# borangundogan/PPO-2DGrid

Hardware: AMD Instinct MI355X
Metric: env-steps/sec (rollout+GAE+PPO update), 4096 envs, 16x16 mediumhard (higher is better)
Workload: dtype fp32

## Files before the change

include/merlin_hip.h:

```cpp
#ifndef MERLIN_HIP_H
#define MERLIN_HIP_H

#include <stdint.h>

#ifdef __cplusplus
extern "C" {
#endif

#define MERLIN_ABI_VERSION 3

#define MERLIN_OK 0
#define MERLIN_E_INVALID 1
#define MERLIN_E_HIP 2
#define MERLIN_E_DEVICE 3
#define MERLIN_E_UNSUPPORTED 4

#define MERLIN_EASY 0
#define MERLIN_MEDIUM 1
#define MERLIN_MEDIUMHARD 2
#define MERLIN_HARD 3
#define MERLIN_HARDEST 4

#define MERLIN_DEVERR_BAD_ACTION 1u
#define MERLIN_DEVERR_PLACE_OBJ 2u
// ... 42 lines not shown
                    double *ep_return_dev, int32_t *ep_length_dev, int32_t autoreset,
                    void *stream);
int merlin_env_act_step(merlin_env *env, const float *head_part_dev, int32_t n_parts, const float *b_actor_dev,
                        const float *b_critic_dev, int32_t act_dim, int32_t deterministic, uint64_t seed,
                        const int64_t *epoch_dev, int64_t step, int64_t env_offset, int64_t *action_dev,
                        float *logp_dev, float *value_dev, uint32_t *obs_dev, float *reward_dev,
                        uint8_t *terminated_dev, uint8_t *truncated_dev, float *done_dev, double *ep_return_dev,
                        int32_t *ep_length_dev, void *stream);
int merlin_group_act(const uint32_t *codes_dev, int32_t groups, const float *T2_dev, const float *b2_dev,
                     const float *W3t_dev, const float *b3_dev, const float *W4p_dev, const float *b4_dev,
                     const float *Wa_dev, const float *ba_dev, const float *Wc_dev, const float *bc_dev,
                     int32_t act_dim, float *a3_ws_dev, float *head_part_dev, int32_t shared_weights, void *stream);
int merlin_env_set_refill_interval(merlin_env *env, int32_t every);
int merlin_env_refill(merlin_env *env, void *stream);
int merlin_env_set_step_fallback(merlin_env *env, int32_t on);
int merlin_env_full_obs(merlin_env *env, uint8_t *out_dev, void *stream);
int merlin_env_get_state(merlin_env *env, uint32_t *walls_host, int32_t *agent_host,
                         uint64_t *rng_host, void *stream);
#define MERLIN_FRAME_TILES 22
int merlin_frame_atlas(int32_t tile_size, uint8_t *out_host);
int merlin_render_frames(const uint32_t *walls_dev, const int32_t *goal_dev, const int32_t *agent_dev,
                         const int32_t *map_index_dev, int64_t n_frames, int32_t size, int32_t tile_size,
                         int32_t highlight, uint8_t *out_dev, void *stream);
int merlin_env_render(merlin_env *env, const int64_t *index_dev, int64_t n, int32_t tile_size,
                      int32_t highlight, uint8_t *out_dev, void *stream);
int merlin_env_snapshot(merlin_env *env, uint32_t *walls_dev, int32_t *goal_dev, int32_t *agent_dev,
                        void *stream);
int merlin_shortest_paths(const uint32_t *walls_dev, const int32_t *goal_dev, const int32_t *agent_dev,
                          const int32_t *map_index_dev, int64_t n, int32_t size, int32_t *dist_dev,
                          int16_t *field_dev, void *stream);
// ... 264 lines not shown
```

ppo-2dgrid_amd/csrc/merlin_capi.hip:

```cpp
#include <math.h>
#include <string.h>

#include <mutex>
#include <string>
#include <vector>

#include <algorithm>

#include "merlin_internal.h"

struct merlin_env {
    merlin::EnvDev dev;
    int device;
    bool has_state;
    int steps_since_refill;
    int refill_every;
    bool no_fallback = false;
    bool seed_slots_full = false;
    uint8_t *diff_buf = nullptr;
};

namespace {

thread_local std::string g_err;
// ... 438 lines not shown
        if (err == hipSuccess) err = hipMemset(*p, 0, bytes);
    };
    alloc((void **)&d.walls, n * d.sp * sizeof(uint32_t));
    alloc((void **)&d.agent, n * sizeof(uint4));
    alloc((void **)&d.rng_s, n * sizeof(ulonglong2));
    alloc((void **)&d.rng_i, n * sizeof(ulonglong2));
    alloc((void **)&d.rng_b, n * sizeof(uint2));
    alloc((void **)&d.ep_ret, n * sizeof(double));
    alloc((void **)&d.ep_len, n * sizeof(int32_t));
    alloc((void **)&d.err, 2 * sizeof(uint32_t));
    alloc((void **)&d.pg_walls, n * d.sp * sizeof(uint32_t));
    alloc((void **)&d.pg_agent, n * sizeof(uint4));
    alloc((void **)&d.pg_rng_s, n * sizeof(ulonglong2));
    alloc((void **)&d.pg_rng_b, n * sizeof(uint2));
    alloc((void **)&d.pg_valid, n * sizeof(uint8_t));
    alloc((void **)&d.rflag, n * sizeof(uint8_t));
    alloc((void **)&d.bflag, (n + 63) / 64);
    if (d.explore_on) alloc((void **)&d.visited, n * d.sp * sizeof(uint32_t));
    alloc((void **)&e->diff_buf, n * sizeof(uint8_t));
    if (err != hipSuccess) {
        merlin_env_destroy(e);
        return hip_fail(err, "hipMalloc(env state)");
    }
    *out = e;
    return MERLIN_OK;
}

int merlin_env_destroy(merlin_env *e) {
    if (!e) return MERLIN_OK;
    merlin::EnvDev &d = e->dev;
    void *ptrs[] = {d.walls, d.agent, d.rng_s, d.rng_i, d.rng_b, d.ep_ret, d.ep_len, d.err, d.visited,
                    d.pg_walls, d.pg_agent, d.pg_rng_s, d.pg_rng_b, d.pg_valid, d.rflag, d.bflag, e->diff_buf};
    for (void *p : ptrs)
        if (p) (void)hipFree(p);
    delete e;
    return MERLIN_OK;
}

int merlin_env_num_envs(const merlin_env *e) { return e ? e->dev.n : -1; }
int merlin_env_size(const merlin_env *e) { return e ? e->dev.size : -1; }

int merlin_env_seed(merlin_env *e, const uint64_t *seeds, int32_t n, void *stream) {
    if (!e || !seeds) return fail(MERLIN_E_INVALID, "null argument");
    if (n != e->dev.n) return fail(MERLIN_E_INVALID, "seed count must equal num_envs");
    hipStream_t s = (hipStream_t)stream;
    const size_t N = (size_t)n;
    ulonglong2 *st = new ulonglong2[N];
    ulonglong2 *inc = new ulonglong2[N];
    for (size_t i = 0; i < N; i++) {
        U128 a, b;
        seed_pcg64(seeds[i], a, b);
        st[i] = make_ulonglong2(a.lo, a.hi);
        inc[i] = make_ulonglong2(b.lo, b.hi);
    }
    hipError_t err = hipMemcpyAsync(e->dev.rng_s, st, N * sizeof(ulonglong2), hipMemcpyHostToDevice, s);
    if (err == hipSuccess)
        err = hipMemcpyAsync(e->dev.rng_i, inc, N * sizeof(ulonglong2), hipMemcpyHostToDevice, s);
    if (err == hipSuccess) err = merlin::zero_async(e->dev.rng_b, N * sizeof(uint2), s);
    if (err == hipSuccess) err = merlin::zero_async(e->dev.pg_valid, N, s);
    e->seed_slots_full = false;
    if (err == hipSuccess) err = hipStreamSynchronize(s);
    delete[] st;
    delete[] inc;
    if (err != hipSuccess) return hip_fail(err, "merlin_env_seed");
    return MERLIN_OK;
}

int merlin_env_set_difficulties(merlin_env *e, const int32_t *diff, int32_t n, void *stream) {
    if (!e) return fail(MERLIN_E_INVALID, "null env");
    hipStream_t s = (hipStream_t)stream;
    const size_t N = (size_t)e->dev.n;
    hipError_t err = hipSuccess;
    uint8_t *host = nullptr;
    if (diff) {
        if (n != e->dev.n) return fail(MERLIN_E_INVALID, "difficulty count must equal num_envs");
        for (size_t i = 0; i < N; i++) {
            if (diff[i] < MERLIN_EASY || diff[i] > MERLIN_HARDEST) return fail(MERLIN_E_INVALID, "unknown difficulty");
            if (diff[i] == MERLIN_HARDEST && e->dev.size < 8)
                return fail(MERLIN_E_UNSUPPORTED, "hardest needs size >= 8 (integers(2, size/2 - 1) is empty below)");
        }
        host = new uint8_t[N];
        for (size_t i = 0; i < N; i++) host[i] = (uint8_t)diff[i];
        err = hipMemcpyAsync(e->diff_buf, host, N, hipMemcpyHostToDevice, s);
        e->dev.diff = e->diff_buf;
    } else {
        e->dev.diff = nullptr;
    }
    if (err == hipSuccess) err = merlin::zero_async(e->dev.pg_valid, N, s);
    e->seed_slots_full = false;
    if (err == hipSuccess) err = hipStreamSynchronize(s);
    delete[] host;
    if (err != hipSuccess) return hip_fail(err, "merlin_env_set_difficulties");
    return MERLIN_OK;
}

int merlin_env_reset(merlin_env *e, const uint8_t *mask, uint32_t *obs, void *stream) {
    if (!e) return fail(MERLIN_E_INVALID, "null env");
    HIP_TRY(merlin::launch_env_reset(e->dev, mask, obs, (hipStream_t)stream));
    e->steps_since_refill = 0;
    if (!mask) {
        e->has_state = true;
        e->seed_slots_full = e->dev.reseed != 0;
    }
    return MERLIN_OK;
}

int merlin_env_step(merlin_env *e, const int64_t *actions, int32_t n_steps, int64_t action_stride,
                    uint32_t *obs, float *reward, uint8_t *term, uint8_t *trunc, float *done,
                    double *ep_ret, int32_t *ep_len, int32_t autoreset, void *stream) {
    if (!e || !actions) return fail(MERLIN_E_INVALID, "null argument");
    if (!e->has_state) return fail(MERLIN_E_INVALID, "merlin_env_step before merlin_env_reset");
    if (n_steps <= 0) return MERLIN_OK;
    if (action_stride < e->dev.n && n_steps > 1)
        return fail(MERLIN_E_INVALID, "action_stride must be >= num_envs");
    merlin::StepOut o{};
    o.actions = actions;
    o.action_stride = action_stride;
// ... 62 lines not shown
    if (!e) return fail(MERLIN_E_INVALID, "null env");
    e->no_fallback = on == 0;
    return MERLIN_OK;
}

int merlin_env_set_refill_interval(merlin_env *e, int32_t every) {
    if (!e) return fail(MERLIN_E_INVALID, "null env");
    if (every < 0) return fail(MERLIN_E_INVALID, "refill interval must be >= 0");
    e->refill_every = every;
    e->steps_since_refill = 0;
    return MERLIN_OK;
}

int merlin_env_refill(merlin_env *e, void *stream) {
    if (!e) return fail(MERLIN_E_INVALID, "null env");
    HIP_TRY(merlin::launch_env_refill(e->dev, false, (hipStream_t)stream));
    return MERLIN_OK;
}

int merlin_env_full_obs(merlin_env *e, uint8_t *out, void *stream) {
    if (!e || !out) return fail(MERLIN_E_INVALID, "null argument");
    HIP_TRY(merlin::launch_env_full_obs(e->dev, out, (hipStream_t)stream));
    return MERLIN_OK;
}

int merlin_env_get_state(merlin_env *e, uint32_t *walls, int32_t *agent, uint64_t *rng, void *stream) {
    if (!e) return fail(MERLIN_E_INVALID, "null env");
    hipStream_t s = (hipStream_t)stream;
    const merlin::EnvDev &d = e->dev;
    const size_t n = (size_t)d.n;
    if (walls) {
// ... 859 lines not shown
```

ppo-2dgrid_amd/csrc/merlin_env.hip:

```cpp
#include <algorithm>

#include <cstdlib>

#include "merlin_internal.h"

namespace merlin {
namespace {

constexpr int BLK = 64;
constexpr int SBLK = 128;
static_assert(SBLK % BLK == 0 && SBLK >= 64, "step blocks: whole waves; one bflag each (merlin_capi.hip: n / 64)");

struct Rng {
    uint64_t slo, shi, ilo, ihi;
    uint32_t has, buf;
};

__device__ __forceinline__ uint64_t rng_peek64(const Rng &r, uint64_t &nlo, uint64_t &hi) {
    const uint64_t MLO = 0x4385df649fccf645ULL, MHI = 0x2360ed051fc65da4ULL;
    const uint64_t lo = r.slo * MLO;
    hi = __umul64hi(r.slo, MLO) + r.slo * MHI + r.shi * MLO;
    nlo = lo + r.ilo;
    hi += r.ihi + (nlo < lo ? 1ULL : 0ULL);
    const uint64_t x = hi ^ nlo;
// ... 438 lines not shown
__device__ __forceinline__ uint4 pack_agent(int ax, int ay, int dir, int steps, int gx, int gy,
                                            int lx, int ly, int stay) {
    return make_uint4((uint32_t)ax | ((uint32_t)ay << 8) | ((uint32_t)dir << 16), (uint32_t)steps,
                      (uint32_t)gx | ((uint32_t)gy << 8),
                      (uint32_t)lx | ((uint32_t)ly << 8) | ((uint32_t)min(stay, 65535) << 16));
}

template <int SP>
__device__ __forceinline__ void reset_visited(const EnvDev &E, int i, int ax, int ay) {
    uint32_t *vis = E.visited + (size_t)i * SP;
    for (int y = 0; y < SP; y++) vis[y] = (y == ay) ? (1u << ax) : 0u;
}

template <int SP, int NB>
__device__ __forceinline__ bool take_slot(const EnvDev &E, int i, uint32_t (*rows)[NB], int lane, GenOut &g) {
    if (!E.pg_valid[i]) return false;
    {
        const uint4 *src = reinterpret_cast<const uint4 *>(E.pg_walls + (size_t)i * SP);
#pragma unroll
        for (int q = 0; q < SP / 4; q++) {
            const uint4 v = src[q];
            rows[4 * q + 0][lane] = v.x;
            rows[4 * q + 1][lane] = v.y;
            rows[4 * q + 2][lane] = v.z;
            rows[4 * q + 3][lane] = v.w;
        }
        const uint4 a = E.pg_agent[i];
        g.ax = a.x & 0xff;
        g.ay = (a.x >> 8) & 0xff;
        g.dir = (a.x >> 16) & 3;
        g.gx = a.z & 0xff;
        g.gy = (a.z >> 8) & 0xff;
        g.err = 0u;
        if (!E.reseed) {
            E.rng_s[i] = E.pg_rng_s[i];
            E.rng_b[i] = E.pg_rng_b[i];
            E.pg_valid[i] = 0;
        }
    }
    return true;
}

__device__ __forceinline__ int env_difficulty(const EnvDev &E, int i) { return E.diff ? (int)E.diff[i] : E.difficulty; }

template <int SP, int NB, bool INL>
__device__ __forceinline__ void take_map(const EnvDev &E, int i, uint32_t (*rows)[NB], int lane, GenOut &g) {
    if (!take_slot<SP, NB>(E, i, rows, lane, g)) {
        Rng r = load_rng(E, i);
        if (INL)
            generate_map_inl<SP, NB>(rows, lane, E.size, env_difficulty(E, i), r, E.err + 1, g);
        else
// ... 19 lines not shown
}

template <int SP>
__global__ __launch_bounds__(BLK) void k_env_reset(EnvDev E, const uint8_t *__restrict__ mask,
                                                  uint32_t *__restrict__ obs) {
    __shared__ uint32_t rows[SP][BLK];
    const int lane = threadIdx.x;
    const int i = blockIdx.x * BLK + lane;
    if (i >= E.n) return;
    if (mask && !mask[i]) return;
    reset_one<SP>(E, i, rows, lane, obs);
}

template <int SP>
__device__ __forceinline__ void refill_one(const EnvDev &E, int i, uint32_t (*rows)[BLK], int lane) {
    Rng r = load_rng(E, i);
    GenOut g;
    generate_map_inl<SP, BLK>(rows, lane, E.size, env_difficulty(E, i), r, E.err + 1, g);
    uint4 *dst = reinterpret_cast<uint4 *>(E.pg_walls + (size_t)i * SP);
#pragma unroll
    for (int q = 0; q < SP / 4; q++) {
        const int y = 4 * q;
        dst[q] = make_uint4(y + 0 < E.size ? rows[y + 0][lane] : 0u, y + 1 < E.size ? rows[y + 1][lane] : 0u,
                            y + 2 < E.size ? rows[y + 2][lane] : 0u, y + 3 < E.size ? rows[y + 3][lane] : 0u);
    }
    E.pg_agent[i] = pack_agent(g.ax, g.ay, g.dir, 0, g.gx, g.gy, g.ax, g.ay, 0);
    E.pg_rng_s[i] = make_ulonglong2(r.slo, r.shi);
    E.pg_rng_b[i] = make_uint2(r.has, r.buf);
    E.pg_valid[i] = 1;
    if (g.err) atomicOr(E.err, g.err);
}

template <int SP, int SPAN>
__global__ __launch_bounds__(BLK) void k_env_refill(EnvDev E) {
    __shared__ uint32_t rows[SP][BLK];
    __shared__ int queue[BLK];
    const int lane = threadIdx.x;
    const unsigned long long below = (1ull << lane) - 1ull;
    static_assert(SPAN == 1 || SPAN == 4 || SPAN == 16, "refill span");
    const int64_t base = ((int64_t)blockIdx.x * BLK + lane) * SPAN;
    uint32_t fl[4] = {0x01010101u, 0x01010101u, 0x01010101u, 0x01010101u};
    if (SPAN == 16 && base + SPAN <= E.n) {
        const uint4 v = *reinterpret_cast<const uint4 *>(E.pg_valid + base);
        fl[0] = v.x;
        fl[1] = v.y;
// ... 206 lines not shown
}

template <int SP>
static hipError_t launch_refill_sp(const EnvDev &E, bool full, hipStream_t s) {
    if (full)
        hipLaunchKernelGGL((k_env_refill<SP, 1>), dim3((E.n + BLK - 1) / BLK), dim3(BLK), 0, s, E);
    else
        hipLaunchKernelGGL((k_env_refill<SP, 4>), dim3((E.n + BLK * 4 - 1) / (BLK * 4)), dim3(BLK), 0, s, E);
    return hipGetLastError();
}

hipError_t launch_env_refill(const EnvDev &E, bool full, hipStream_t s) {
    return E.sp == 16 ? launch_refill_sp<16>(E, full, s) : launch_refill_sp<32>(E, full, s);
}

hipError_t launch_env_reset(const EnvDev &E, const uint8_t *mask, uint32_t *obs, hipStream_t s) {
    const dim3 grid((E.n + BLK - 1) / BLK), block(BLK);
    if (E.sp == 16)
        hipLaunchKernelGGL(k_env_reset<16>, grid, block, 0, s, E, mask, obs);
    else
        hipLaunchKernelGGL(k_env_reset<32>, grid, block, 0, s, E, mask, obs);
    hipError_t e = hipGetLastError();
    return e != hipSuccess ? e : launch_env_refill(E, mask == nullptr, s);
}

template <int SP>
static hipError_t launch_step_sp(const EnvDev &E, const StepOut &O, hipStream_t s) {
    const int nb = (E.n + SBLK - 1) / SBLK;
    if (!O.autoreset) {
        hipLaunchKernelGGL((k_env_step<SP, true>), dim3(nb), dim3(SBLK), 0, s, E, O);
    } else if (O.n_steps == 1) {
        if (O.act.part)
            hipLaunchKernelGGL((k_env_step<SP, true, true>), dim3(nb), dim3(SBLK), 0, s, E, O);
        else
            hipLaunchKernelGGL((k_env_step<SP, true>), dim3(nb), dim3(SBLK), 0, s, E, O);
        hipError_t e = hipGetLastError();
        if (e != hipSuccess) return e;
        if (!O.no_fallback)
// ... 21 lines not shown
```

ppo-2dgrid_amd/csrc/merlin_internal.h:

```cpp
#pragma once

#include <hip/hip_runtime.h>
#include <stdint.h>

#include "merlin_hip.h"

namespace merlin {

struct EnvDev {
    int n, size, sp, difficulty, max_steps;
    int stuck_on, max_stay;
    double penalty;
    int explore_on;
    double bonus;
    int reseed;
    uint32_t *walls;
    uint4 *agent;
    ulonglong2 *rng_s;
    ulonglong2 *rng_i;
    uint2 *rng_b;
    double *ep_ret;
    int32_t *ep_len;
    uint32_t *visited;
    uint32_t *err;
    uint32_t *pg_walls;
    uint4 *pg_agent;
    ulonglong2 *pg_rng_s;
    uint2 *pg_rng_b;
    uint8_t *pg_valid;
    uint8_t *rflag;
    uint8_t *bflag;
    const uint8_t *diff;
};

constexpr int REFILL_EVERY = 16;

constexpr int ACT_MAXA = 8;
constexpr int ACT_PARTS_UNROLL = 8;


__device__ __forceinline__ float relu_nan(float v) { return v != v ? v : fmaxf(v, 0.0f); }

__device__ __forceinline__ uint64_t mix64(uint64_t x) {
    x ^= x >> 30;
// ... 197 lines not shown
};

hipError_t zero_async(void *p, size_t bytes, hipStream_t s);
hipError_t launch_group_act(const uint32_t *codes, int G, const float *T2, const float *b2, const float *W3t,
                            const float *b3, const float *W4p, const float *b4, const float *Wa, const float *ba,
                            const float *Wc, const float *bc, int A, float *a3, float *part, bool shared, hipStream_t s);
hipError_t launch_h3p_gemm_nt(const void *A, const uint32_t *amaxA, const void *B, const uint32_t *amaxB, int64_t M,
                              int N, int K, int T, int64_t a_stride, int64_t b_stride, const float *bias, float *C,
                              int64_t c_stride, int cfg, hipStream_t s, const int32_t *a_rows = nullptr,
                              const float *head_w0 = nullptr, int n_actions = 0, const float *head_w1 = nullptr,
                              float *head_part = nullptr);
void set_h3p_walk_blocks(int n);
hipError_t launch_h3p_gemm_tn_gather(const void *A, const uint32_t *amaxA, const void *B, const uint32_t *amaxB,
                                     int64_t Kd, int M, int N, int T, int64_t a_stride, int64_t b_stride, int splits,
                                     float *slab, const int32_t *b_rows, int cfg, int *S_out, hipStream_t s);
hipError_t launch_env_reset(const EnvDev &E, const uint8_t *mask, uint32_t *obs, hipStream_t s);
hipError_t launch_env_step(const EnvDev &E, const StepOut &O, bool refill, hipStream_t s);
hipError_t launch_env_full_obs(const EnvDev &E, uint8_t *out, hipStream_t s);
hipError_t launch_env_refill(const EnvDev &E, bool full, hipStream_t s);
hipError_t upload_atlas(const uint8_t *atlas_host);
hipError_t launch_render_frames(const uint32_t *walls, const int32_t *goal, const int32_t *agent,
                                const int32_t *map_index, int64_t n_frames, int size, int ts, int highlight,
                                const uint8_t *atlas, uint8_t *out, uint32_t *err, hipStream_t s);
hipError_t launch_env_render(const EnvDev &E, const int64_t *index, int64_t n_frames, int ts, int highlight,
                             const uint8_t *atlas, uint8_t *out, hipStream_t s);
hipError_t launch_env_snapshot(const EnvDev &E, uint32_t *walls, int32_t *goal, int32_t *agent, hipStream_t s);
hipError_t launch_shortest_paths(const uint32_t *walls, const int32_t *goal, const int32_t *agent,
                                 const int32_t *map_index, int64_t n, int size, int32_t *dist, int16_t *field,
                                 hipStream_t s);
hipError_t launch_env_optimal_steps(const EnvDev &E, int32_t *dist, int16_t *field, hipStream_t s);
void shortest_paths_host(const uint32_t *walls, const int32_t *goal, const int32_t *agent, int64_t n, int S,
// ... 209 lines not shown
```

ppo-2dgrid_amd/merlin/_native.py:

```python
from __future__ import annotations

import contextlib
import ctypes as C
import gc
import os

import torch

PKG_ROOT = os.path.dirname(os.path.dirname(os.path.abspath(__file__)))
LIB_PATH = os.environ.get("MERLIN_HIP_LIB", os.path.join(PKG_ROOT, "lib", "libmerlin_hip.so"))

MERLIN_OK = 0
E_INVALID, E_HIP, E_DEVICE, E_UNSUPPORTED = 1, 2, 3, 4
LAYOUT_NCHW = 0
LAYOUT_NHWC = 1
OBS_WORDS = 8
DEVERR_BAD_ACTION = 1
DEVERR_PLACE_OBJ = 2
DEVERR_BAD_TILE = 4
DEVERR_SLOT_EMPTY = 8
DEVERR_BAD_FRAME = 16
FRAME_TILES = 22

DIFFICULTY_IDS = {"easy": 0, "medium": 1, "mediumhard": 2, "hard": 3, "hardest": 4}
# ... 43 lines not shown
    L.merlin_tile_atlas.argtypes = [vp]
    L.merlin_env_config_layout.argtypes = [C.POINTER(C.c_int64), i32]
    L.merlin_env_config_layout.restype = i64
    L.merlin_env_create.argtypes = [C.POINTER(EnvConfig), C.POINTER(vp)]
    L.merlin_env_destroy.argtypes = [vp]
    L.merlin_env_seed.argtypes = [vp, u64p, i32, vp]
    L.merlin_env_set_difficulties.argtypes = [vp, C.POINTER(C.c_int32), i32, vp]
    L.merlin_env_reset.argtypes = [vp, vp, vp, vp]
    L.merlin_env_step.argtypes = [vp, vp, i32, i64, vp, vp, vp, vp, vp, vp, vp, i32, vp]
    L.merlin_group_act.argtypes = [vp, i32, vp, vp, vp, vp, vp, vp, vp, vp, vp, vp, i32, vp, vp, i32, vp]
    L.merlin_env_act_step.argtypes = [vp, vp, i32, vp, vp, i32, i32, C.c_uint64, vp, i64, i64, vp, vp, vp, vp, vp,
                                      vp, vp, vp, vp, vp, vp]
    L.merlin_env_set_refill_interval.argtypes = [vp, i32]
    L.merlin_env_set_step_fallback.argtypes = [vp, i32]
    L.merlin_env_refill.argtypes = [vp, vp]
    L.merlin_env_get_state.argtypes = [vp, vp, vp, vp, vp]
    L.merlin_env_full_obs.argtypes = [vp, vp, vp]
    L.merlin_env_errors.argtypes = [vp, C.POINTER(C.c_uint32), C.POINTER(C.c_uint32), vp]
    L.merlin_obs_expand_f32.argtypes = [vp, vp, i64, vp, C.c_float, i32, vp]
    L.merlin_obs_expand_u8.argtypes = [vp, vp, i64, vp, vp]
    L.merlin_gae.argtypes = [vp, vp, vp, vp, vp, vp, i32, i32, C.c_double, C.c_double, vp, vp]
    L.merlin_adv_normalize.argtypes = [vp, i64, vp, vp, vp]
    L.merlin_conv1_lut_fwd.argtypes = [vp, vp, i64, vp, vp, i32, vp, vp]
    L.merlin_conv1_lut_bwd.argtypes = [vp, vp, i64, vp, vp, i32, vp, vp, vp]
    L.merlin_tower_conv2_im2col_fwd.argtypes = [vp, vp, i64, vp, vp, i32, vp, vp]
    L.merlin_tower_conv2_im2col_bwd.argtypes = [vp, vp, i64, vp, vp, vp, i32, vp, vp, vp]
    L.merlin_tower_conv3_im2col_fwd.argtypes = [vp, vp, i64, i32, vp, vp]
    L.merlin_tower_conv3_col2im_bwd.argtypes = [vp, vp, vp, i64, i32, vp, vp]
    L.merlin_tower_conv3_col2im_bwd_chunked.argtypes = [vp, vp, vp, i64, i32, vp, vp, vp]
    L.merlin_tower_conv2_lut_rows.restype = C.c_int
# ... 100 lines not shown
    size = int(L.merlin_env_config_layout(offs, nf))
    return size, [int(o) for o in offs]


def check_env_config_layout(L) -> None:
    size, offs = env_config_layout(L)
    mine = [getattr(EnvConfig, f).offset for f, _ in EnvConfig._fields_]
    if size != C.sizeof(EnvConfig) or offs != mine:
        raise MerlinNativeError(f"EnvConfig layout mismatch: C sizeof {size} offsets {offs}, "
                                f"ctypes sizeof {C.sizeof(EnvConfig)} offsets {mine}")


EXPORTED_SYMBOLS = (
    "merlin_version", "merlin_last_error", "merlin_tile_atlas", "merlin_env_config_layout", "merlin_env_create",
    "merlin_env_destroy", "merlin_env_seed", "merlin_env_reset", "merlin_env_step", "merlin_env_act_step", "merlin_group_act",
    "merlin_env_set_refill_interval", "merlin_env_refill",
    "merlin_env_get_state", "merlin_env_full_obs", "merlin_env_errors", "merlin_env_set_step_fallback", "merlin_env_num_envs", "merlin_env_size",
    "merlin_obs_expand_f32", "merlin_obs_expand_u8", "merlin_gae", "merlin_adv_normalize",
    "merlin_conv1_lut_fwd", "merlin_conv1_lut_bwd", "merlin_tower_conv2_im2col_fwd",
    "merlin_tower_conv2_im2col_bwd", "merlin_tower_conv3_im2col_fwd", "merlin_tower_conv3_col2im_bwd",
    "merlin_tower_conv3_col2im_bwd_chunked", "merlin_tower_conv2_lut_rows", "merlin_tower_conv2_lut_fwd",
    "merlin_tower_conv2_lut_bwd", "merlin_tower_conv2_lut_fwd_grouped", "merlin_tower_conv2_lut_slab_bytes",
    "merlin_tower_conv2_lut_bwd_grouped", "merlin_tower_window_lut", "merlin_tower_window_lut_bias_relu", "merlin_minibatch_patch_maps", "merlin_segment_sum_mask_rows", "merlin_tower_window_conv3",
    "merlin_tower_window_conv3_bits", "merlin_tower_window_conv3_reuse", "merlin_tower_all_windows", "merlin_tower_codes_conv3",
    "merlin_tower_codes_conv3_amax", "merlin_tower_errors",
    "merlin_segment_sum", "merlin_segment_sum_masked", "merlin_segment_sum_marked", "merlin_segment_sum_fused", "merlin_tower_heads_fwd", "merlin_tower_bias_relu", "merlin_tower_relu_bwd", "merlin_tower_head_bwd",
    "merlin_tower_colsum",
    "merlin_ppo_loss_workspace", "merlin_ppo_loss", "merlin_act_heads",
    "merlin_x6_split", "merlin_x6_join", "merlin_x6_gemm_nt", "merlin_x6_tn_slab_floats", "merlin_x6_gemm_tn",
    "merlin_clip_adam_workspace", "merlin_clip_adam",
    "merlin_h3_amax", "merlin_h3_split", "merlin_h3_gemm_nt", "merlin_h3_gemm_tn",
# ... 1334 lines not shown
```

ppo-2dgrid_amd/merlin/envs.py:

```python
from __future__ import annotations

import ctypes as C
import os

import numpy as np
import torch

from . import _native as nat


class Discrete:

    def __init__(self, n: int):
        self.n = n
        self.shape = ()
        self.dtype = np.int64

    def sample(self):
        return int(np.random.randint(self.n))


class Box:
    def __init__(self, low, high, shape, dtype):
        self.low, self.high, self.shape, self.dtype = low, high, tuple(shape), dtype
# ... 30 lines not shown
        self.fully_observable, self.flatten = bool(fully_observable), bool(flatten)
        shape = (self.size, self.size, 3) if self.fully_observable else (56, 56, 3)
        if self.flatten:
            shape = (int(np.prod(shape)),)
        self.single_observation_space = Box(0, 255, shape, np.uint8)
        self.observation_space = self.single_observation_space
        cfg = nat.EnvConfig(self.num_envs, self.size, nat.DIFFICULTY_IDS[uniform], self.max_steps,
                            int(stuck_penalty), int(max_stay), float(penalty), int(exploration_bonus),
                            float(bonus), int(reseed_each_reset))
        self._lib = nat.lib()
        nat.drain_deferred()
        with torch.cuda.device(self.device):
            h = C.c_void_p()
            nat.check(self._lib.merlin_env_create(C.byref(cfg), C.byref(h)), "merlin_env_create")
        self._h = h
        self.class_ids = torch.full((self.num_envs,), nat.DIFFICULTY_IDS[uniform], dtype=torch.uint8,
                                    device=self.device)
        self.per_env_classes = False
        self.uniform_difficulty = uniform
        if names is not None:
            self.set_difficulties(names)
        self._seed_pending = seed
        self._seeded_once = False
        if seeds is not None:
            self.seed_each(seeds)
        self.obs = torch.zeros((self.num_envs, nat.OBS_WORDS), dtype=torch.int32, device=self.device)
        n = self.num_envs
        self._rew = torch.zeros(n, dtype=torch.float32, device=self.device)
        self._term = torch.zeros(n, dtype=torch.uint8, device=self.device)
        self._trunc = torch.zeros(n, dtype=torch.uint8, device=self.device)
# ... 6 lines not shown
            self._h = None
            lib_ = self._lib
            nat.defer_release(lambda: lib_.merlin_env_destroy(h))

    def __del__(self):
        try:
            self.close()
        except Exception:
            pass

    @property
    def _stream(self):
        return C.c_void_p(torch.cuda.current_stream(self.device).cuda_stream)

    def seed(self, seed: int) -> None:
        seeds = (np.arange(self.num_envs, dtype=np.uint64) + np.uint64(self.env_offset)
                 + np.uint64(seed))
        with torch.cuda.device(self.device):
            nat.check(self._lib.merlin_env_seed(self._h, seeds.ctypes.data_as(C.POINTER(C.c_uint64)),
                                                self.num_envs, self._stream), "merlin_env_seed")
        self._seeded_once = True

    def set_base_seed(self, seed: int) -> None:
        self._seed_pending = int(seed)
        self._seeded_once = False

    def seed_each(self, seeds) -> None:
        seeds = np.ascontiguousarray(np.asarray(seeds, dtype=np.uint64))
        assert seeds.shape == (self.num_envs,)
        with torch.cuda.device(self.device):
            nat.check(self._lib.merlin_env_seed(self._h, seeds.ctypes.data_as(C.POINTER(C.c_uint64)),
                                                self.num_envs, self._stream), "merlin_env_seed")
        self._seeded_once = True

    def _check_names(self, names) -> list:
        names = [str(d) for d in names]
        if len(names) != self.num_envs:
            raise ValueError(f"difficulty: {len(names)} names for {self.num_envs} envs")
        for d in names:
            if d not in nat.DIFFICULTY_IDS:
                raise ValueError(f"Unknown difficulty: {d}")
        return names

    def set_difficulties(self, names) -> None:
        if names is None:
            with torch.cuda.device(self.device):
                nat.check(self._lib.merlin_env_set_difficulties(self._h, None, 0, self._stream),
                          "merlin_env_set_difficulties")
            self.per_env_classes = False
            self.difficulty, self.difficulties = self.uniform_difficulty, [self.uniform_difficulty] * self.num_envs
            self.class_ids.fill_(nat.DIFFICULTY_IDS[self.uniform_difficulty])
            return
        names = self._check_names(names)
        self.set_class_ids(np.array([nat.DIFFICULTY_IDS[d] for d in names], dtype=np.int32))

    def set_class_ids(self, ids) -> None:
        ids = np.ascontiguousarray(np.asarray(ids, dtype=np.int32))
        with torch.cuda.device(self.device):
            nat.check(self._lib.merlin_env_set_difficulties(self._h, ids.ctypes.data_as(C.POINTER(C.c_int32)),
                                                            int(ids.size), self._stream),
                      "merlin_env_set_difficulties")
        inv = {v: k for k, v in nat.DIFFICULTY_IDS.items()}
        self.difficulties = [inv[int(v)] for v in ids]
        self.difficulty = self.difficulties[0] if len(set(self.difficulties)) == 1 else "mixed"
        self.class_ids.copy_(torch.from_numpy(ids.astype(np.uint8)))
        self.per_env_classes = True

    def reset(self, seed: int | None = None, mask: torch.Tensor | None = None, out: torch.Tensor | None = None):
        if seed is None and not self._seeded_once:
            seed = self._seed_pending if self._seed_pending is not None else _entropy_seed()
        if seed is not None:
            self.seed(seed)
        out = self.obs if out is None else out
        if mask is not None:
            mask = mask.to(torch.uint8).contiguous()
            if out.data_ptr() != self.obs.data_ptr():
                out.copy_(self.obs)
        with torch.cuda.device(self.device):
            nat.check(self._lib.merlin_env_reset(self._h, nat.ptr(mask), nat.ptr(out), self._stream),
                      "merlin_env_reset")
        if out.data_ptr() != self.obs.data_ptr():
            self.obs.copy_(out)
        return out

    def step_into(self, actions: torch.Tensor, obs_out: torch.Tensor | None = None, reward=None, term=None,
                  trunc=None, done=None, ep_return=None, ep_length=None, n_steps: int = 1,
                  action_stride: int | None = None, autoreset: bool = True) -> None:
        assert actions.dtype == torch.int64 and actions.is_contiguous()
        stride = self.num_envs if action_stride is None else int(action_stride)
        with torch.cuda.device(self.device), nat.KernelTimer.span("k_env_step", self.num_envs * n_steps * ENV_STEP_BYTES):
            nat.check(self._lib.merlin_env_step(
                self._h, nat.ptr(actions), int(n_steps), stride, nat.ptr(obs_out), nat.ptr(reward),
                nat.ptr(term), nat.ptr(trunc), nat.ptr(done), nat.ptr(ep_return), nat.ptr(ep_length),
                int(bool(autoreset)), self._stream), "merlin_env_step")

    def act_step_into(self, part: torch.Tensor, b_actor: torch.Tensor, b_critic: torch.Tensor, out, obs_out=None,
                      reward=None, term=None, trunc=None, done=None, ep_return=None, ep_length=None,
                      deterministic: bool = False, seed: int = 0, epoch=None, step: int = 0) -> None:
        action, logp, value = out
        P = int(part.shape[1])
        A = int(b_actor.numel())
        assert part.dtype == torch.float32 and part.is_contiguous() and part.shape == (2, P, self.num_envs, 4)
        assert action.dtype == torch.int64 and action.numel() == logp.numel() == value.numel() == self.num_envs
        assert b_critic.numel() == 1 and 1 <= A <= 4
        if not deterministic and epoch is None:
            raise ValueError("act_step_into: a sampled action needs an epoch counter tensor (int64[1] on the device)")
        with torch.cuda.device(self.device), nat.KernelTimer.span("k_env_step", self.num_envs * ENV_STEP_BYTES):
            nat.check(self._lib.merlin_env_act_step(
                self._h, nat.ptr(part), P, nat.ptr(b_actor), nat.ptr(b_critic), A, int(bool(deterministic)),
                int(seed) & 0xFFFFFFFFFFFFFFFF, nat.ptr(epoch), int(step), int(self.env_offset), nat.ptr(action),
                nat.ptr(logp), nat.ptr(value), nat.ptr(obs_out), nat.ptr(reward), nat.ptr(term), nat.ptr(trunc),
                nat.ptr(done), nat.ptr(ep_return), nat.ptr(ep_length), self._stream), "merlin_env_act_step")

    def set_refill_interval(self, every: int) -> None:
        nat.check(self._lib.merlin_env_set_refill_interval(self._h, int(every)), "merlin_env_set_refill_interval")

    def set_step_fallback(self, on: bool) -> None:
        nat.check(self._lib.merlin_env_set_step_fallback(self._h, 1 if on else 0), "merlin_env_set_step_fallback")

    def refill(self) -> None:
        with torch.cuda.device(self.device):
            nat.check(self._lib.merlin_env_refill(self._h, self._stream), "merlin_env_refill")

    def step(self, actions: torch.Tensor, autoreset: bool = True):
        actions = actions.to(device=self.device, dtype=torch.int64).contiguous()
        self.step_into(actions, self.obs, self._rew, self._term, self._trunc, None, self._epr, self._epl,
                       autoreset=autoreset)
        info = {"episode_return": self._epr, "episode_length": self._epl}
        return self.obs, self._rew, self._term.bool(), self._trunc.bool(), info

    def render_obs(self, codes: torch.Tensor | None = None, index: torch.Tensor | None = None,
                   out: torch.Tensor | None = None, scale: float = 1.0, layout: str = "nchw"):
        codes = self.obs if codes is None else codes
        return nat.expand_obs(codes.reshape(-1, nat.OBS_WORDS), index=index, out=out, scale=scale,
                              layout=layout)

    def render_rgb(self, codes: torch.Tensor | None = None) -> torch.Tensor:
# ... 165 lines not shown
```

ppo-2dgrid_amd/merlin/ppo.py:

```python
from __future__ import annotations

import time

import warnings

import numpy as np
import torch
import torch.optim as optim

from . import _native as nat
from .actor_critic import CNNActorCritic, MLPActorCritic
from .distributed import DataParallel
from .envs import MerlinEnv, MerlinVecEnv
from .metrics.ppo_metrics import aggregate_ppo_update_metrics
from .rollout_buffer import CodeRolloutBuffer, RolloutBuffer
from .windows import deferred_fc1_wgrad

INV255 = 1.0 / 255.0


class _PPOLoss(torch.autograd.Function):

    @staticmethod
    def forward(ctx, logits, value, bias_actor, bias_critic, mb, sample_index, actions, logp_old, adv, ret, clip_eps,
                vf_coef, ent_coef, stats):
        loss, dlogits, dvalue, dba, dbc = nat.ppo_loss(
            logits.detach(), value.detach(), mb.offs, mb.order, mb.inv, sample_index, actions, logp_old, adv, ret,
            clip_eps, vf_coef, ent_coef, stats, bias_actor=bias_actor, bias_critic=bias_critic)
        ctx.save_for_backward(dlogits, dvalue, dba, dbc.view_as(bias_critic))
        return loss

    @staticmethod
    def backward(ctx, g):
        return tuple(d * g for d in ctx.saved_tensors) + (None,) * 10


ROLLOUT_SCALE_ROWS = True
FUSE_ACT_STEP = True
ROLLOUT_STEP_FALLBACK = False


class PPO:
    def __init__(self, env, lr=3e-4, gamma=0.99, lam=0.95, clip_eps=0.2, update_epochs=10,
                 batch_size=2048, minibatch_size=256, vf_coef=0.5, ent_coef=0.01, device="cuda",
                 *, dp: DataParallel | None = None, perm_fn=None, conv1_from_codes: bool = True,
                 dedup: bool = True, windows: bool = True, rollout_graph: bool = True):
        self.env = env
        self.device = torch.device(device)
        if self.device.type != "cuda":
            raise nat.MerlinNativeError("merlin.PPO runs its hot path as HIP kernels; pass a GPU device")
        self.gamma, self.lam, self.clip_eps = gamma, lam, clip_eps
        self.update_epochs = update_epochs
        self.minibatch_size = minibatch_size
        self.vf_coef, self.ent_coef = vf_coef, ent_coef
# ... 34 lines not shown
                self.conv1_from_codes = False
                if getattr(self.vec, "fully_observable", False):
                    self._full_obs = torch.empty((self.k_steps + 1, N) + self.obs_shape, dtype=torch.uint8,
                                                 device=self.device)
            elif getattr(self.vec, "fully_observable", False):
                raise ValueError("the full grid without flatten is smaller than CNNActorCritic's receptive field")
            else:
                self.use_cnn = True
                self.obs_shape = (56, 56, 3)
                self.ac = CNNActorCritic(self.obs_shape, act_dim).to(self.device)
            self.buf = CodeRolloutBuffer(self.k_steps, N, self.device)
            self._obs_step = torch.empty((N, 3, 56, 56), dtype=torch.float32, device=self.device)
            self._mb_obs = None
            self._refill_stream = (torch.cuda.Stream(self.device) if self.device.type == "cuda" and self.use_cnn
                                   else None)
            if self._refill_stream is not None:
                self.vec.set_refill_interval(0)
        else:
            sample_obs, _ = env.reset()
            self.num_envs, self.k_steps, self.batch_size = 1, batch_size, batch_size
            if sample_obs.ndim == 1:
                self.use_cnn = False
                self.obs_shape = (int(np.prod(sample_obs.shape)),)
                self.ac = MLPActorCritic(self.obs_shape[0], act_dim).to(self.device)
            else:
                self.use_cnn = True
                self.obs_shape = sample_obs.shape
                self.ac = CNNActorCritic(self.obs_shape, act_dim).to(self.device)
            self.buffer = RolloutBuffer(batch_size, self.obs_shape, self.device, is_discrete=True)
        from .fast_step import flatten_parameters

        self._flat_params = flatten_parameters(self.ac)
# ... 19 lines not shown
        off, base = 0, self._flat_params.data_ptr()
        for p in self.ac.parameters():
            if p.data_ptr() != base + p.element_size() * off:
                return False
            off += p.numel()
        return off == self._flat_params.numel()

    def _rehome_parameters(self) -> None:
        from .fast_step import flatten_parameters

        torch.cuda.synchronize(self.device)
        self._graph = None
        self._wstep = None
        self._flat_params = flatten_parameters(self.ac)

    def collect_rollouts(self):
        if self.vec is None:
            return self._collect_rollouts_single()
        if not self.use_cnn:
            return self._collect_rollouts_flat()
        if self._graph is not None and not self._params_on_flat():
            self._rehome_parameters()
        if self._graph is not None:
            self._graph.replay()
        else:
            self._rollout_body()
            if self.rollout_graph and self.conv1_from_codes:
                self._capture_rollout()
        self._record_episodes()
        self.vec.errors()
        if self.rollout_all_windows:
            nat.tower_errors(self.device)
        lv = self.buf.last_value
        return float(lv[0].item()) if self.num_envs == 1 else lv

    def _rollout_body(self):
        buf, env = self.buf, self.vec
        T = buf.T
        main, side = torch.cuda.current_stream(self.device), self._refill_stream
        every = max(1, int(self.refill_every))
        env.set_step_fallback(ROLLOUT_STEP_FALLBACK or side is None or every != 1)
        env.reset(out=buf.codes[0])
        with torch.no_grad():
            self._act_epoch.add_(1)
            if self.conv1_from_codes and self.rollout_all_windows is None:
                self.rollout_all_windows = self.ac._use_all_windows((T + 1) * buf.N, self.device)
            pack = (self.ac.rollout_pack(frames=(T + 1) * buf.N, all_windows=self.rollout_all_windows,
                                         steps=T + 1 if ROLLOUT_SCALE_ROWS else None)
                    if self.conv1_from_codes else None)
            pending = False
            fused = FUSE_ACT_STEP and pack is not None and self.ac.heads_partials_ok(pack)
            for t in range(T):
                if fused:
                    part = self.ac.act_codes_packed(buf.codes[t], pack, step=t, partials=True)
                else:
                    self._act(buf.codes[t], pack, t, out=(buf.actions[t], buf.logprobs[t], buf.values[t]))
# ... 5 lines not shown
                                      (buf.actions[t], buf.logprobs[t], buf.values[t]), buf.codes[t + 1],
                                      buf.rewards[t], None, None, buf.dones[t], buf.ep_return[t], buf.ep_length[t],
                                      seed=self._act_seed, epoch=self._act_epoch, step=t)
                else:
                    env.step_into(buf.actions[t], buf.codes[t + 1], buf.rewards[t], None, None, buf.dones[t],
                                  buf.ep_return[t], buf.ep_length[t])
                if side is not None and (t % every == every - 1 or t == T - 1):
                    side.wait_stream(main)
                    with torch.cuda.stream(side):
                        env.refill()
                    pending = True
            _, _, last_value = self._act(buf.codes[T], pack, T)
            if pending:
                main.wait_stream(side)
            buf.last_value.copy_(last_value)

    def _capture_rollout(self):
        torch.cuda.synchronize(self.device)
        g = torch.cuda.CUDAGraph()
        try:
            with nat.capture_guard(), torch.cuda.graph(g):
                self._rollout_body()
        except Exception as e:
            warnings.warn(f"rollout graph capture failed, rollouts stay eager: {e}")
            self.rollout_graph = False
            torch.cuda.synchronize(self.device)
            return
        self._graph = g

    def _act(self, codes, pack, step, out=None):
# ... 232 lines not shown
```

Before: 4.654 million.

## Pre-generate a per-env ring of future maps on a side stream across rollouts

Adds a per-env ring buffer of pre-generated maps, depth k_steps+1, so every reset needed during a rollout can be served from maps generated ahead of time. The top-up refill is launched on a side stream after each rollout so it can overlap the GAE/PPO update, replacing the per-step refill launches and stream waits inside the rollout loop. This costs extra device memory, capped by a 1 GiB budget, and adds ring bookkeeping in the slot-take and refill kernels. Any change to seeding or difficulty drops the ring.

```diff
diff --git a/include/merlin_hip.h b/include/merlin_hip.h
--- a/include/merlin_hip.h
+++ b/include/merlin_hip.h
@@ -80,6 +80,7 @@
 int merlin_env_set_refill_interval(merlin_env *env, int32_t every);
 int merlin_env_refill(merlin_env *env, void *stream);
 int merlin_env_set_step_fallback(merlin_env *env, int32_t on);
+int merlin_env_set_lookahead_depth(merlin_env *env, int32_t depth);
 int merlin_env_full_obs(merlin_env *env, uint8_t *out_dev, void *stream);
 int merlin_env_get_state(merlin_env *env, uint32_t *walls_host, int32_t *agent_host,
                          uint64_t *rng_host, void *stream);
diff --git a/ppo-2dgrid_amd/csrc/merlin_capi.hip b/ppo-2dgrid_amd/csrc/merlin_capi.hip
--- a/ppo-2dgrid_amd/csrc/merlin_capi.hip
+++ b/ppo-2dgrid_amd/csrc/merlin_capi.hip
@@ -476,6 +476,8 @@
     alloc((void **)&d.pg_rng_s, n * sizeof(ulonglong2));
     alloc((void **)&d.pg_rng_b, n * sizeof(uint2));
     alloc((void **)&d.pg_valid, n * sizeof(uint8_t));
+    alloc((void **)&d.pg_ring, n * sizeof(uint32_t));
+    d.pg_depth = 1;
     alloc((void **)&d.rflag, n * sizeof(uint8_t));
     alloc((void **)&d.bflag, (n + 63) / 64);
     if (d.explore_on) alloc((void **)&d.visited, n * d.sp * sizeof(uint32_t));
@@ -492,7 +494,8 @@
     if (!e) return MERLIN_OK;
     merlin::EnvDev &d = e->dev;
     void *ptrs[] = {d.walls, d.agent, d.rng_s, d.rng_i, d.rng_b, d.ep_ret, d.ep_len, d.err, d.visited,
-                    d.pg_walls, d.pg_agent, d.pg_rng_s, d.pg_rng_b, d.pg_valid, d.rflag, d.bflag, e->diff_buf};
+                    d.pg_walls, d.pg_agent, d.pg_rng_s, d.pg_rng_b, d.pg_valid, d.pg_ring, d.rflag, d.bflag,
+                    e->diff_buf};
     for (void *p : ptrs)
         if (p) (void)hipFree(p);
     delete e;
@@ -501,6 +504,14 @@
 
 int merlin_env_num_envs(const merlin_env *e) { return e ? e->dev.n : -1; }
 int merlin_env_size(const merlin_env *e) { return e ? e->dev.size : -1; }
+
+static hipError_t drop_lookahead(merlin_env *e, hipStream_t s) {
+    const size_t N = (size_t)e->dev.n;
+    hipError_t err = merlin::zero_async(e->dev.pg_valid, N, s);
+    if (err == hipSuccess) err = merlin::zero_async(e->dev.pg_ring, N * sizeof(uint32_t), s);
+    e->seed_slots_full = false;
+    return err;
+}
 
 int merlin_env_seed(merlin_env *e, const uint64_t *seeds, int32_t n, void *stream) {
     if (!e || !seeds) return fail(MERLIN_E_INVALID, "null argument");
@@ -519,7 +530,7 @@
     if (err == hipSuccess)
         err = hipMemcpyAsync(e->dev.rng_i, inc, N * sizeof(ulonglong2), hipMemcpyHostToDevice, s);
     if (err == hipSuccess) err = merlin::zero_async(e->dev.rng_b, N * sizeof(uint2), s);
-    if (err == hipSuccess) err = merlin::zero_async(e->dev.pg_valid, N, s);
+    if (err == hipSuccess) err = drop_lookahead(e, s);
     e->seed_slots_full = false;
     if (err == hipSuccess) err = hipStreamSynchronize(s);
     delete[] st;
@@ -548,7 +559,7 @@
     } else {
         e->dev.diff = nullptr;
     }
-    if (err == hipSuccess) err = merlin::zero_async(e->dev.pg_valid, N, s);
+    if (err == hipSuccess) err = drop_lookahead(e, s);
     e->seed_slots_full = false;
     if (err == hipSuccess) err = hipStreamSynchronize(s);
     delete[] host;
@@ -558,11 +569,12 @@
 
 int merlin_env_reset(merlin_env *e, const uint8_t *mask, uint32_t *obs, void *stream) {
     if (!e) return fail(MERLIN_E_INVALID, "null env");
-    HIP_TRY(merlin::launch_env_reset(e->dev, mask, obs, (hipStream_t)stream));
+    const bool refill = e->dev.pg_depth == 1 || e->refill_every > 0;
+    HIP_TRY(merlin::launch_env_reset(e->dev, mask, obs, refill, (hipStream_t)stream));
     e->steps_since_refill = 0;
     if (!mask) {
         e->has_state = true;
-        e->seed_slots_full = e->dev.reseed != 0;
+        e->seed_slots_full = e->dev.reseed != 0 && refill;
     }
     return MERLIN_OK;
 }
@@ -655,7 +667,39 @@
 
 int merlin_env_refill(merlin_env *e, void *stream) {
     if (!e) return fail(MERLIN_E_INVALID, "null env");
-    HIP_TRY(merlin::launch_env_refill(e->dev, false, (hipStream_t)stream));
+    HIP_TRY(merlin::launch_env_refill(e->dev, e->dev.pg_depth > 1, (hipStream_t)stream));
+    return MERLIN_OK;
+}
+
+int merlin_env_set_lookahead_depth(merlin_env *e, int32_t depth) {
+    if (!e) return fail(MERLIN_E_INVALID, "null env");
+    if (depth < 1 || depth > 65535) return fail(MERLIN_E_INVALID, "look-ahead depth must be in [1, 65535]");
+    merlin::EnvDev &d = e->dev;
+    HIP_TRY(hipDeviceSynchronize());
+    const size_t slots = (size_t)d.n * (size_t)depth;
+    void *p[4] = {nullptr, nullptr, nullptr, nullptr};
+    const size_t bytes[4] = {slots * d.sp * sizeof(uint32_t), slots * sizeof(uint4), slots * sizeof(ulonglong2),
+                             slots * sizeof(uint2)};
+    hipError_t err = hipSuccess;
+    for (int k = 0; k < 4 && err == hipSuccess; k++) {
+        err = hipMalloc(&p[k], bytes[k]);
+        if (err == hipSuccess) err = hipMemset(p[k], 0, bytes[k]);
+    }
+    if (err != hipSuccess) {
+        for (void *q : p)
+            if (q) (void)hipFree(q);
+        return hip_fail(err, "hipMalloc(look-ahead ring)");
+    }
+    void *old[4] = {d.pg_walls, d.pg_agent, d.pg_rng_s, d.pg_rng_b};
+    for (void *q : old) (void)hipFree(q);
+    d.pg_walls = (uint32_t *)p[0];
+    d.pg_agent = (uint4 *)p[1];
+    d.pg_rng_s = (ulonglong2 *)p[2];
+    d.pg_rng_b = (uint2 *)p[3];
+    d.pg_depth = depth;
+    e->steps_since_refill = 0;
+    HIP_TRY(drop_lookahead(e, nullptr));
+    HIP_TRY(hipStreamSynchronize(nullptr));
     return MERLIN_OK;
 }
 
diff --git a/ppo-2dgrid_amd/csrc/merlin_env.hip b/ppo-2dgrid_amd/csrc/merlin_env.hip
--- a/ppo-2dgrid_amd/csrc/merlin_env.hip
+++ b/ppo-2dgrid_amd/csrc/merlin_env.hip
@@ -476,9 +476,11 @@
 
 template <int SP, int NB>
 __device__ __forceinline__ bool take_slot(const EnvDev &E, int i, uint32_t (*rows)[NB], int lane, GenOut &g) {
-    if (!E.pg_valid[i]) return false;
+    const uint32_t ring = E.pg_ring[i], head = ring & 0xffffu, count = ring >> 16;
+    if (!count) return false;
     {
-        const uint4 *src = reinterpret_cast<const uint4 *>(E.pg_walls + (size_t)i * SP);
+        const size_t k = (size_t)i * E.pg_depth + head;
+        const uint4 *src = reinterpret_cast<const uint4 *>(E.pg_walls + k * SP);
 #pragma unroll
         for (int q = 0; q < SP / 4; q++) {
             const uint4 v = src[q];
@@ -487,7 +489,7 @@
             rows[4 * q + 2][lane] = v.z;
             rows[4 * q + 3][lane] = v.w;
         }
-        const uint4 a = E.pg_agent[i];
+        const uint4 a = E.pg_agent[k];
         g.ax = a.x & 0xff;
         g.ay = (a.x >> 8) & 0xff;
         g.dir = (a.x >> 16) & 3;
@@ -495,8 +497,9 @@
         g.gy = (a.z >> 8) & 0xff;
         g.err = 0u;
         if (!E.reseed) {
-            E.rng_s[i] = E.pg_rng_s[i];
-            E.rng_b[i] = E.pg_rng_b[i];
+            E.rng_s[i] = E.pg_rng_s[k];
+            E.rng_b[i] = E.pg_rng_b[k];
+            E.pg_ring[i] = (head + 1 == (uint32_t)E.pg_depth ? 0u : head + 1) | ((count - 1) << 16);
             E.pg_valid[i] = 0;
         }
     }
@@ -546,21 +549,43 @@
 
 template <int SP>
 __device__ __forceinline__ void refill_one(const EnvDev &E, int i, uint32_t (*rows)[BLK], int lane) {
+    const int D = E.pg_depth, want = E.reseed ? 1 : D;
+    const uint32_t ring = E.pg_ring[i];
+    const int head = (int)(ring & 0xffffu);
+    int count = (int)(ring >> 16);
     Rng r = load_rng(E, i);
-    GenOut g;
-    generate_map_inl<SP, BLK>(rows, lane, E.size, env_difficulty(E, i), r, E.err + 1, g);
-    uint4 *dst = reinterpret_cast<uint4 *>(E.pg_walls + (size_t)i * SP);
-#pragma unroll
-    for (int q = 0; q < SP / 4; q++) {
-        const int y = 4 * q;
-        dst[q] = make_uint4(y + 0 < E.size ? rows[y + 0][lane] : 0u, y + 1 < E.size ? rows[y + 1][lane] : 0u,
-                            y + 2 < E.size ? rows[y + 2][lane] : 0u, y + 3 < E.size ? rows[y + 3][lane] : 0u);
-    }
-    E.pg_agent[i] = pack_agent(g.ax, g.ay, g.dir, 0, g.gx, g.gy, g.ax, g.ay, 0);
-    E.pg_rng_s[i] = make_ulonglong2(r.slo, r.shi);
-    E.pg_rng_b[i] = make_uint2(r.has, r.buf);
+    if (count) {
+        const int last = head + count - 1;
+        const size_t k = (size_t)i * D + (last >= D ? last - D : last);
+        const ulonglong2 s = E.pg_rng_s[k];
+        const uint2 b = E.pg_rng_b[k];
+        r.slo = s.x;
+        r.shi = s.y;
+        r.has = b.x;
+        r.buf = b.y;
+    }
+    const int difficulty = env_difficulty(E, i);
+    uint32_t err = 0u;
+    for (; count < want; count++) {
+        const int slot = head + count;
+        const size_t k = (size_t)i * D + (slot >= D ? slot - D : slot);
+        GenOut g;
+        generate_map_inl<SP, BLK>(rows, lane, E.size, difficulty, r, E.err + 1, g);
+        uint4 *dst = reinterpret_cast<uint4 *>(E.pg_walls + k * SP);
+#pragma unroll
+        for (int q = 0; q < SP / 4; q++) {
+            const int y = 4 * q;
+            dst[q] = make_uint4(y + 0 < E.size ? rows[y + 0][lane] : 0u, y + 1 < E.size ? rows[y + 1][lane] : 0u,
+                                y + 2 < E.size ? rows[y + 2][lane] : 0u, y + 3 < E.size ? rows[y + 3][lane] : 0u);
+        }
+        E.pg_agent[k] = pack_agent(g.ax, g.ay, g.dir, 0, g.gx, g.gy, g.ax, g.ay, 0);
+        E.pg_rng_s[k] = make_ulonglong2(r.slo, r.shi);
+        E.pg_rng_b[k] = make_uint2(r.has, r.buf);
+        err |= g.err;
+    }
+    E.pg_ring[i] = (uint32_t)head | ((uint32_t)count << 16);
     E.pg_valid[i] = 1;
-    if (g.err) atomicOr(E.err, g.err);
+    if (err) atomicOr(E.err, err);
 }
 
 template <int SP, int SPAN>
@@ -797,14 +822,14 @@
     return E.sp == 16 ? launch_refill_sp<16>(E, full, s) : launch_refill_sp<32>(E, full, s);
 }
 
-hipError_t launch_env_reset(const EnvDev &E, const uint8_t *mask, uint32_t *obs, hipStream_t s) {
+hipError_t launch_env_reset(const EnvDev &E, const uint8_t *mask, uint32_t *obs, bool refill, hipStream_t s) {
     const dim3 grid((E.n + BLK - 1) / BLK), block(BLK);
     if (E.sp == 16)
         hipLaunchKernelGGL(k_env_reset<16>, grid, block, 0, s, E, mask, obs);
     else
         hipLaunchKernelGGL(k_env_reset<32>, grid, block, 0, s, E, mask, obs);
     hipError_t e = hipGetLastError();
-    return e != hipSuccess ? e : launch_env_refill(E, mask == nullptr, s);
+    return (e != hipSuccess || !refill) ? e : launch_env_refill(E, mask == nullptr, s);
 }
 
 template <int SP>
diff --git a/ppo-2dgrid_amd/csrc/merlin_internal.h b/ppo-2dgrid_amd/csrc/merlin_internal.h
--- a/ppo-2dgrid_amd/csrc/merlin_internal.h
+++ b/ppo-2dgrid_amd/csrc/merlin_internal.h
@@ -28,6 +28,8 @@
     ulonglong2 *pg_rng_s;
     uint2 *pg_rng_b;
     uint8_t *pg_valid;
+    uint32_t *pg_ring;
+    int pg_depth;
     uint8_t *rflag;
     uint8_t *bflag;
     const uint8_t *diff;
@@ -255,7 +257,7 @@
 hipError_t launch_h3p_gemm_tn_gather(const void *A, const uint32_t *amaxA, const void *B, const uint32_t *amaxB,
                                      int64_t Kd, int M, int N, int T, int64_t a_stride, int64_t b_stride, int splits,
                                      float *slab, const int32_t *b_rows, int cfg, int *S_out, hipStream_t s);
-hipError_t launch_env_reset(const EnvDev &E, const uint8_t *mask, uint32_t *obs, hipStream_t s);
+hipError_t launch_env_reset(const EnvDev &E, const uint8_t *mask, uint32_t *obs, bool refill, hipStream_t s);
 hipError_t launch_env_step(const EnvDev &E, const StepOut &O, bool refill, hipStream_t s);
 hipError_t launch_env_full_obs(const EnvDev &E, uint8_t *out, hipStream_t s);
 hipError_t launch_env_refill(const EnvDev &E, bool full, hipStream_t s);
diff --git a/ppo-2dgrid_amd/merlin/_native.py b/ppo-2dgrid_amd/merlin/_native.py
--- a/ppo-2dgrid_amd/merlin/_native.py
+++ b/ppo-2dgrid_amd/merlin/_native.py
@@ -81,6 +81,7 @@
     L.merlin_env_set_refill_interval.argtypes = [vp, i32]
     L.merlin_env_set_step_fallback.argtypes = [vp, i32]
     L.merlin_env_refill.argtypes = [vp, vp]
+    L.merlin_env_set_lookahead_depth.argtypes = [vp, i32]
     L.merlin_env_get_state.argtypes = [vp, vp, vp, vp, vp]
     L.merlin_env_full_obs.argtypes = [vp, vp, vp]
     L.merlin_env_errors.argtypes = [vp, C.POINTER(C.c_uint32), C.POINTER(C.c_uint32), vp]
@@ -211,7 +212,7 @@
 EXPORTED_SYMBOLS = (
     "merlin_version", "merlin_last_error", "merlin_tile_atlas", "merlin_env_config_layout", "merlin_env_create",
     "merlin_env_destroy", "merlin_env_seed", "merlin_env_reset", "merlin_env_step", "merlin_env_act_step", "merlin_group_act",
-    "merlin_env_set_refill_interval", "merlin_env_refill",
+    "merlin_env_set_refill_interval", "merlin_env_refill", "merlin_env_set_lookahead_depth",
     "merlin_env_get_state", "merlin_env_full_obs", "merlin_env_errors", "merlin_env_set_step_fallback", "merlin_env_num_envs", "merlin_env_size",
     "merlin_obs_expand_f32", "merlin_obs_expand_u8", "merlin_gae", "merlin_adv_normalize",
     "merlin_conv1_lut_fwd", "merlin_conv1_lut_bwd", "merlin_tower_conv2_im2col_fwd",
diff --git a/ppo-2dgrid_amd/merlin/envs.py b/ppo-2dgrid_amd/merlin/envs.py
--- a/ppo-2dgrid_amd/merlin/envs.py
+++ b/ppo-2dgrid_amd/merlin/envs.py
@@ -68,6 +68,9 @@
             h = C.c_void_p()
             nat.check(self._lib.merlin_env_create(C.byref(cfg), C.byref(h)), "merlin_env_create")
         self._h = h
+        self.lookahead_depth = 1
+        self.step_fallback = True
+        self._topup = None
         self.class_ids = torch.full((self.num_envs,), nat.DIFFICULTY_IDS[uniform], dtype=torch.uint8,
                                     device=self.device)
         self.per_env_classes = False
@@ -104,6 +107,7 @@
         return C.c_void_p(torch.cuda.current_stream(self.device).cuda_stream)
 
     def seed(self, seed: int) -> None:
+        self.join_refill()
         seeds = (np.arange(self.num_envs, dtype=np.uint64) + np.uint64(self.env_offset)
                  + np.uint64(seed))
         with torch.cuda.device(self.device):
@@ -118,6 +122,7 @@
     def seed_each(self, seeds) -> None:
         seeds = np.ascontiguousarray(np.asarray(seeds, dtype=np.uint64))
         assert seeds.shape == (self.num_envs,)
+        self.join_refill()
         with torch.cuda.device(self.device):
             nat.check(self._lib.merlin_env_seed(self._h, seeds.ctypes.data_as(C.POINTER(C.c_uint64)),
                                                 self.num_envs, self._stream), "merlin_env_seed")
@@ -133,6 +138,7 @@
         return names
 
     def set_difficulties(self, names) -> None:
+        self.join_refill()
         if names is None:
             with torch.cuda.device(self.device):
                 nat.check(self._lib.merlin_env_set_difficulties(self._h, None, 0, self._stream),
@@ -146,6 +152,7 @@
 
     def set_class_ids(self, ids) -> None:
         ids = np.ascontiguousarray(np.asarray(ids, dtype=np.int32))
+        self.join_refill()
         with torch.cuda.device(self.device):
             nat.check(self._lib.merlin_env_set_difficulties(self._h, ids.ctypes.data_as(C.POINTER(C.c_int32)),
                                                             int(ids.size), self._stream),
@@ -156,11 +163,15 @@
         self.class_ids.copy_(torch.from_numpy(ids.astype(np.uint8)))
         self.per_env_classes = True
 
+    def ensure_seeded(self) -> None:
+        if not self._seeded_once:
+            self.seed(self._seed_pending if self._seed_pending is not None else _entropy_seed())
+
     def reset(self, seed: int | None = None, mask: torch.Tensor | None = None, out: torch.Tensor | None = None):
-        if seed is None and not self._seeded_once:
-            seed = self._seed_pending if self._seed_pending is not None else _entropy_seed()
+        self.join_refill()
         if seed is not None:
             self.seed(seed)
+        self.ensure_seeded()
         out = self.obs if out is None else out
         if mask is not None:
             mask = mask.to(torch.uint8).contiguous()
@@ -178,6 +189,7 @@
                   action_stride: int | None = None, autoreset: bool = True) -> None:
         assert actions.dtype == torch.int64 and actions.is_contiguous()
         stride = self.num_envs if action_stride is None else int(action_stride)
+        self.join_refill()
         with torch.cuda.device(self.device), nat.KernelTimer.span("k_env_step", self.num_envs * n_steps * ENV_STEP_BYTES):
             nat.check(self._lib.merlin_env_step(
                 self._h, nat.ptr(actions), int(n_steps), stride, nat.ptr(obs_out), nat.ptr(reward),
@@ -195,6 +207,7 @@
         assert b_critic.numel() == 1 and 1 <= A <= 4
         if not deterministic and epoch is None:
             raise ValueError("act_step_into: a sampled action needs an epoch counter tensor (int64[1] on the device)")
+        self.join_refill()
         with torch.cuda.device(self.device), nat.KernelTimer.span("k_env_step", self.num_envs * ENV_STEP_BYTES):
             nat.check(self._lib.merlin_env_act_step(
                 self._h, nat.ptr(part), P, nat.ptr(b_actor), nat.ptr(b_critic), A, int(bool(deterministic)),
@@ -207,10 +220,36 @@
 
     def set_step_fallback(self, on: bool) -> None:
         nat.check(self._lib.merlin_env_set_step_fallback(self._h, 1 if on else 0), "merlin_env_set_step_fallback")
-
-    def refill(self) -> None:
-        with torch.cuda.device(self.device):
+        self.step_fallback = bool(on)
+
+    def set_lookahead_depth(self, depth: int) -> None:
+        self.join_refill()
+        with torch.cuda.device(self.device):
+            nat.check(self._lib.merlin_env_set_lookahead_depth(self._h, int(depth)), "merlin_env_set_lookahead_depth")
+        self.lookahead_depth = int(depth)
+
+    def lookahead_bytes(self, depth: int) -> int:
+        return self.num_envs * int(depth) * (4 * (16 if self.size <= 16 else 32) + 40)
+
+    def refill(self, stream=None) -> None:
+        self.join_refill()
+        if stream is None:
+            with torch.cuda.device(self.device):
+                nat.check(self._lib.merlin_env_refill(self._h, self._stream), "merlin_env_refill")
+            return
+        stream.wait_stream(torch.cuda.current_stream(self.device))
+        with torch.cuda.device(self.device), torch.cuda.stream(stream):
             nat.check(self._lib.merlin_env_refill(self._h, self._stream), "merlin_env_refill")
+        self._topup = stream
+
+    @property
+    def refill_pending(self) -> bool:
+        return self._topup is not None
+
+    def join_refill(self) -> None:
+        if self._topup is not None:
+            torch.cuda.current_stream(self.device).wait_stream(self._topup)
+            self._topup = None
 
     def step(self, actions: torch.Tensor, autoreset: bool = True):
         actions = actions.to(device=self.device, dtype=torch.int64).contiguous()
diff --git a/ppo-2dgrid_amd/merlin/ppo.py b/ppo-2dgrid_amd/merlin/ppo.py
--- a/ppo-2dgrid_amd/merlin/ppo.py
+++ b/ppo-2dgrid_amd/merlin/ppo.py
@@ -38,6 +38,8 @@
 ROLLOUT_SCALE_ROWS = True
 FUSE_ACT_STEP = True
 ROLLOUT_STEP_FALLBACK = False
+ROLLOUT_MAP_RING = True
+ROLLOUT_RING_BUDGET = 1 << 30
 
 
 class PPO:
@@ -102,8 +104,10 @@
             self._mb_obs = None
             self._refill_stream = (torch.cuda.Stream(self.device) if self.device.type == "cuda" and self.use_cnn
                                    else None)
+            self._ring = False
             if self._refill_stream is not None:
                 self.vec.set_refill_interval(0)
+                self.set_map_ring(ROLLOUT_MAP_RING)
         else:
             sample_obs, _ = env.reset()
             self.num_envs, self.k_steps, self.batch_size = 1, batch_size, batch_size
@@ -153,6 +157,18 @@
         self._wstep = None
         self._flat_params = flatten_parameters(self.ac)
 
+    def set_map_ring(self, on: bool) -> bool:
+        if getattr(self, "_refill_stream", None) is None:
+            return False
+        depth = self.k_steps + 1
+        ring = bool(on) and self.vec.lookahead_bytes(depth) <= ROLLOUT_RING_BUDGET
+        if ring != self._ring or self.vec.lookahead_depth != (depth if ring else 1):
+            torch.cuda.synchronize(self.device)
+            self._graph = None
+            self.vec.set_lookahead_depth(depth if ring else 1)
+            self._ring = ring
+        return ring
+
     def collect_rollouts(self):
         if self.vec is None:
             return self._collect_rollouts_single()
@@ -160,6 +176,12 @@
             return self._collect_rollouts_flat()
         if self._graph is not None and not self._params_on_flat():
             self._rehome_parameters()
+        if self._ring:
+            if self.vec.refill_pending:
+                self.vec.join_refill()
+            else:
+                self.vec.ensure_seeded()
+                self.vec.refill()
         if self._graph is not None:
             self._graph.replay()
         else:
@@ -168,6 +190,8 @@
                 self._capture_rollout()
         self._record_episodes()
         self.vec.errors()
+        if self._ring:
+            self.vec.refill(stream=self._refill_stream)
         if self.rollout_all_windows:
             nat.tower_errors(self.device)
         lv = self.buf.last_value
@@ -178,7 +202,12 @@
         T = buf.T
         main, side = torch.cuda.current_stream(self.device), self._refill_stream
         every = max(1, int(self.refill_every))
-        env.set_step_fallback(ROLLOUT_STEP_FALLBACK or side is None or every != 1)
+        fallback_was = env.step_fallback
+        if self._ring:
+            side = None
+            env.set_step_fallback(ROLLOUT_STEP_FALLBACK)
+        else:
+            env.set_step_fallback(ROLLOUT_STEP_FALLBACK or side is None or every != 1)
         env.reset(out=buf.codes[0])
         with torch.no_grad():
             self._act_epoch.add_(1)
@@ -214,6 +243,7 @@
             if pending:
                 main.wait_stream(side)
             buf.last_value.copy_(last_value)
+        env.set_step_fallback(fallback_was)
 
     def _capture_rollout(self):
         torch.cuda.synchronize(self.device)
```

Measured after the change: 4.745 million (median of 6 runs). 2.0% higher.
